# mpieva/mapping-iterative-assembler

Hardware: NVIDIA B200
Metric: aligned reads/sec per iteration (windowed PSSM DP + traceback + score cut + consensus) (higher is better)
Workload: dtype int32

## Files before the change

include/miagpu.h:

```cpp
#ifndef MIAGPU_H
#define MIAGPU_H

#include <stdint.h>

#ifdef __cplusplus
extern "C" {
#endif

#define MIAGPU_MAX_READ      256
#define MIAGPU_PSSM_INTS     775
#define MIAGPU_MAX_RUNS      24
#define MIAGPU_NBUCKET       10
#define MIAGPU_COUNTS_PER_COL 10

#define MIAGPU_RUN_M 0
#define MIAGPU_RUN_I 1
#define MIAGPU_RUN_D 2
#define MIAGPU_RUN_TYPE(x) ((x) >> 14)
#define MIAGPU_RUN_LEN(x)  ((x) & 0x3fff)

#define MIAGPU_ST_OK          0
#define MIAGPU_ST_RUNS_OVERFLOW 1
#define MIAGPU_ST_SKIPPED     2
#define MIAGPU_ST_STR_OVERFLOW 4
// ... 208 lines not shown
  const uint16_t* packed;
  const uint8_t* unique_best;
  const uint8_t* dropped_front;
  const uint8_t* dropped_back;
  const int64_t* fsdb_order;
} miagpu_maln_reads;

int miagpu_maln_ref_size( int ref_len, int circular );
int miagpu_write_maln( const char* path, const miagpu_maln_header* hd,
                       const miagpu_maln_reads* rd, int64_t* n_alnseqs_out );

int miagpu_write_maln_fsdb( miagpu_ctx* ctx, const char* path, const miagpu_maln_header* hd,
                            const miagpu_maln_reads* rd, int64_t* n_alnseqs_out );

#define MIAGPU_MISINC_INTS 1116
int miagpu_misincorporation( miagpu_ctx* ctx, int64_t* counts );

int miagpu_last_buckets( miagpu_ctx* ctx, int32_t* k, int32_t* reads,
                         int64_t* cells, float* ms );
#define MIAGPU_NPAIRCLASS 8
int miagpu_last_pair_buckets( miagpu_ctx* ctx, int32_t* k, int32_t* reads, int32_t* pairs,
                              int64_t* cells, float* ms, int32_t* fallback_reads,
                              int32_t* max_len16 );
int miagpu_last_timing( miagpu_ctx* ctx, float* ms_kernels, float* ms_h2d,
                        float* ms_d2h, int64_t* dp_cells, int32_t* launches );
int miagpu_int32_peak( miagpu_ctx* ctx, double* ops_per_s );
void* miagpu_stream( miagpu_ctx* ctx );

#ifdef __cplusplus
}
#endif
#endif
```

mapping-iterative-assembler_b200/api.py:

```python
import ctypes as C
import os

import numpy as np

HERE = os.path.dirname(os.path.abspath(__file__))
LIB_PATH = os.environ.get("MIAGPU_LIB") or os.path.join(HERE, "libmiagpu.so")
MAX_RUNS = 24
RUN_M, RUN_I, RUN_D = 0, 1, 2
MISINC_SHAPE = (31, 6, 6)
MISINC_CODES = "ACGTN-"

_i32p = C.POINTER(C.c_int32)
_u8p = C.POINTER(C.c_uint8)
_u16p = C.POINTER(C.c_uint16)
_i64p = C.POINTER(C.c_int64)


class MiaGpuError(RuntimeError):
    pass


ENTRY_DTYPE = np.dtype([("read", np.int32), ("col_begin", np.int32), ("col_count", np.int32), ("ref_pos", np.int32),
                        ("front_len", np.int32), ("total_len", np.int32), ("act_bias", np.int32), ("dropped", np.uint8),
                        ("back_formula", np.uint8), ("reserved", np.uint8, 2)])
# ... 40 lines not shown
    L.miagpu_score_cut.argtypes = [C.c_int64, C.c_void_p, C.c_void_p, C.c_void_p, C.POINTER(C.c_double), C.POINTER(C.c_double)]
    L.miagpu_cull_flags.argtypes = [C.c_int64, C.c_void_p, C.c_void_p, C.c_void_p, C.c_int, C.c_int, C.c_double, C.c_double, C.c_void_p]
    L.miagpu_set_alignment_inputs.argtypes = [C.c_void_p, C.c_void_p, C.c_void_p, C.c_void_p]
    L.miagpu_realign_resident.argtypes = [C.c_void_p]
    L.miagpu_adopt_alignment.argtypes = [C.c_void_p, C.c_void_p, C.c_void_p, C.c_void_p]
    L.miagpu_set_cut_inputs.argtypes = [C.c_void_p, C.c_void_p, C.c_void_p, C.c_void_p]
    L.miagpu_reset_dropped.argtypes = [C.c_void_p]
    L.miagpu_iterate_resident.argtypes = [C.c_void_p, C.c_int, C.c_int, C.c_double, C.c_double, C.c_int, C.POINTER(C.c_double),
                                          C.POINTER(C.c_double), C.c_void_p, C.c_void_p, C.c_void_p, _i32p]
    L.miagpu_last_buckets.argtypes = [C.c_void_p, C.c_void_p, C.c_void_p, C.c_void_p, C.c_void_p]
    L.miagpu_iterate_host.argtypes = ([C.c_void_p, C.c_int64] + [C.c_void_p] * 12 + [C.c_int64, _i64p, C.c_void_p, C.c_void_p, C.c_int, C.c_int,
                                      C.c_double, C.c_double, C.c_void_p, C.c_int, C.c_void_p, C.c_char_p, _i32p])
    _vpp = C.POINTER(C.c_void_p)
    L.miagpu_shard_begin.argtypes = [C.c_void_p, C.c_int, C.c_int, C.c_int64, C.c_int, C.c_int, C.c_double, C.c_double, _vpp, _i64p]
    L.miagpu_shard_begin_host.argtypes = ([C.c_void_p, C.c_int, C.c_int, C.c_int64, C.c_int64] + [C.c_void_p] * 14 +
                                          [C.c_int, C.c_int, C.c_double, C.c_double, _vpp, _i64p])
    L.miagpu_shard_fit.argtypes = [C.c_void_p, _vpp, _vpp, _i64p]
    L.miagpu_shard_cut.argtypes = [C.c_void_p, C.POINTER(C.c_double), C.POINTER(C.c_double), _vpp, _i64p]
    L.miagpu_shard_finish.argtypes = [C.c_void_p, C.c_int, C.c_void_p, C.c_void_p, C.c_int64, _i64p, C.c_void_p, C.c_char_p, _i32p]
    L.miagpu_last_cut_stats.argtypes = [C.c_void_p, _i64p, _i64p]
    L.miagpu_trim.argtypes = [C.c_void_p, C.c_int64, C.c_void_p, C.c_void_p, C.c_char_p, C.c_int] + [C.c_void_p] * 6
    L.miagpu_repeat_filter.argtypes = [C.c_void_p, C.c_int64] + [C.c_void_p] * 5 + [C.c_int, C.c_int, C.c_void_p, C.c_void_p]
    L.miagpu_last_pair_buckets.argtypes = [C.c_void_p] + [C.c_void_p] * 5 + [_i32p, _i32p]
    L.miagpu_last_timing.argtypes = [C.c_void_p, C.POINTER(C.c_float), C.POINTER(C.c_float), C.POINTER(C.c_float), _i64p, _i32p]
    L.miagpu_int32_peak.argtypes = [C.c_void_p, C.POINTER(C.c_double)]
    L.miagpu_get_alignment.argtypes = [C.c_void_p] + [C.c_void_p] * 6
    L.miagpu_align_windows.argtypes = [C.c_void_p] + [C.c_void_p] * 3 + [C.c_int] + [C.c_void_p] * 7
    L.miagpu_fastx_open.argtypes = [_vpp, C.c_char_p]
    L.miagpu_fastx_open_memory.argtypes = [_vpp, C.c_void_p, C.c_int64]
    L.miagpu_fastx_format.argtypes = [C.c_void_p]
    L.miagpu_fastx_next.argtypes = [C.c_void_p, C.c_int64, _i64p]
    L.miagpu_fastx_batch.argtypes = [C.c_void_p] + [_vpp] * 7
    L.miagpu_fastx_close.argtypes = [C.c_void_p]
    L.miagpu_fastx_close.restype = None
    L.miagpu_maln_ref_size.argtypes = [C.c_int, C.c_int]
    L.miagpu_read_pssm.argtypes = [C.c_char_p, _i32p]
    L.miagpu_write_maln.argtypes = [C.c_char_p, C.c_void_p, C.c_void_p, _i64p]
    L.miagpu_write_maln_fsdb.argtypes = [C.c_void_p, C.c_char_p, C.c_void_p, C.c_void_p, _i64p]
    L.miagpu_set_fsdb.argtypes = [C.c_void_p] + [C.c_void_p] * 6 + [C.c_int64, C.c_void_p, C.c_int]
    L.miagpu_get_fsdb.argtypes = [C.c_void_p] + [C.c_void_p] * 6 + [_i64p]
    L.miagpu_last_fsdb_stats.argtypes = [C.c_void_p, _i64p, _i64p, _i64p, _i64p]
    L.miagpu_distant_retry.argtypes = [C.c_void_p, _i64p, _i64p]
    L.miagpu_distant_retry_begin.argtypes = [C.c_void_p, _i64p, _i32p]
    L.miagpu_distant_retry_end.argtypes = [C.c_void_p, C.c_int, _i64p]
    L.miagpu_misincorporation.argtypes = [C.c_void_p, _i64p]
    L.miagpu_stream.restype = C.c_void_p
    L.miagpu_stream.argtypes = [C.c_void_p]
    _lib = L
    return L


EXPORTS = ["miagpu_device_count", "miagpu_create", "miagpu_destroy", "miagpu_last_error", "miagpu_version", "miagpu_set_pssm",
           "miagpu_get_pssm", "miagpu_set_reference", "miagpu_ref_wrap_len", "miagpu_build_kmers", "miagpu_upload_reads",
           "miagpu_pass1", "miagpu_last_pass1_stats", "miagpu_last_pass1_route", "miagpu_compact_reads", "miagpu_realign", "miagpu_realign_host", "miagpu_iterate_host", "miagpu_get_runs_packed",
           "miagpu_consensus", "miagpu_accumulate_gaps", "miagpu_accumulate_counts", "miagpu_call", "miagpu_consensus_natural", "miagpu_accumulate_gaps_natural",
           "miagpu_score_cut", "miagpu_cull_flags",
           "miagpu_set_alignment_inputs", "miagpu_realign_resident", "miagpu_adopt_alignment", "miagpu_set_cut_inputs", "miagpu_reset_dropped", "miagpu_iterate_resident", "miagpu_last_buckets", "miagpu_last_pair_buckets", "miagpu_last_timing",
           "miagpu_int32_peak", "miagpu_stream", "miagpu_shard_begin", "miagpu_shard_begin_host", "miagpu_shard_fit", "miagpu_shard_cut", "miagpu_shard_finish",
           "miagpu_last_cut_stats", "miagpu_repeat_filter", "miagpu_trim", "miagpu_get_alignment",
           "miagpu_fastx_open", "miagpu_fastx_open_memory", "miagpu_fastx_format", "miagpu_fastx_next", "miagpu_fastx_batch", "miagpu_fastx_close",
           "miagpu_maln_ref_size", "miagpu_write_maln", "miagpu_read_pssm", "miagpu_align_windows",
           "miagpu_set_fsdb", "miagpu_get_fsdb", "miagpu_last_fsdb_stats", "miagpu_distant_retry", "miagpu_write_maln_fsdb", "miagpu_last_pass1_cells", "miagpu_set_homopolymer", "miagpu_shard_flags", "miagpu_set_cons_capacity",
           "miagpu_distant_retry_begin", "miagpu_distant_retry_end", "miagpu_misincorporation"]


def _ptr(a):
    if a is None:
        return None
    if hasattr(a, "data_ptr"):
        return C.c_void_p(a.data_ptr())
    return C.c_void_p(a.ctypes.data)


class MiaGpu:

    def __init__(self, device=0):
        self.lib = load_library()
        h = C.c_void_p()
        if not self.lib.miagpu_create(C.byref(h), device):
            raise MiaGpuError(self.lib.miagpu_last_error().decode())
# ... 299 lines not shown
        return sc, a, e

    def get_alignment(self):
        out = {k: np.zeros(self.n, np.int32) for k in ("score", "as_out", "ae_out", "abr", "n_runs")}
        out["status"] = np.zeros(self.n, np.uint8)
        self._ck(self.lib.miagpu_get_alignment(self.h, *[_ptr(out[k]) for k in ("score", "as_out", "ae_out", "abr", "n_runs", "status")]))
        return out

    def realign_resident(self):
        self._ck(self.lib.miagpu_realign_resident(self.h))

    def last_buckets(self):
        k, r, cells, ms = np.zeros(10, np.int32), np.zeros(10, np.int32), np.zeros(10, np.int64), np.zeros(10, np.float32)
        self._ck(self.lib.miagpu_last_buckets(self.h, _ptr(k), _ptr(r), _ptr(cells), _ptr(ms)))
        return [dict(K=int(k[i]), reads=int(r[i]), cells=int(cells[i]), ms=float(ms[i])) for i in range(10) if r[i]]

    def last_pair_buckets(self):
        k, r, pr = np.zeros(8, np.int32), np.zeros(8, np.int32), np.zeros(8, np.int32)
        cells, ms = np.zeros(8, np.int64), np.zeros(8, np.float32)
        fb, ml = C.c_int32(), C.c_int32()
        self._ck(self.lib.miagpu_last_pair_buckets(self.h, _ptr(k), _ptr(r), _ptr(pr), _ptr(cells), _ptr(ms), C.byref(fb), C.byref(ml)))
        return ([dict(K=int(k[i]), reads=int(r[i]), pairs=int(pr[i]), cells=int(cells[i]), ms=float(ms[i])) for i in range(8) if r[i]],
                fb.value, ml.value)

    def accumulate_gaps(self, entries):
        entries = np.ascontiguousarray(entries, ENTRY_DTYPE)
        ptr, n = C.c_void_p(), C.c_int64()
        self._ck(self.lib.miagpu_accumulate_gaps(self.h, len(entries), _ptr(entries), C.byref(ptr), C.byref(n)))
        return ptr.value, n.value

    def accumulate_counts(self):
        ptr, n = C.c_void_p(), C.c_int64()
        self._ck(self.lib.miagpu_accumulate_counts(self.h, C.byref(ptr), C.byref(n)))
        return ptr.value, n.value

    def call(self, cons_code=1, want_counts=False, max_len=None):
        gaps = np.zeros(self.seq_len, np.int32)
        counts = np.zeros((self.seq_len, 10), np.int32) if want_counts else None
        buf = C.create_string_buffer(max_len or (self.seq_len * 4 + 4096))
        n = C.c_int32()
        self._ck(self.lib.miagpu_call(self.h, cons_code, _ptr(gaps), _ptr(counts), buf, C.byref(n)))
        return buf.value.decode(), gaps, counts

    def last_timing(self):
        k, h, d = C.c_float(), C.c_float(), C.c_float()
        cells, launches = C.c_int64(), C.c_int32()
# ... 147 lines not shown
```

mapping-iterative-assembler_b200/csrc/miagpu.cu:

```cuda
#include <stdarg.h>
#include <string.h>
#include <stdlib.h>

#include <algorithm>
#include <functional>
#include <chrono>
#include <thread>
#include <vector>

#include "common.cuh"
#include "realign.cuh"
#include "pair16.cuh"
#include "consensus.cuh"
#include "strip.cuh"
#include "pass1.cuh"
#include "sweep16.cuh"
#include "scorecut.hpp"
#include "scorecut.cuh"
#include "repeat.cuh"
#include "slots.cuh"
#include <unordered_map>
#include <cub/device/device_scan.cuh>
#include <cub/device/device_radix_sort.cuh>

namespace miagpu {

static thread_local char g_err[1024] = "";
void set_error(const char* fmt, ...) {
  va_list ap;
  va_start(ap, fmt);
  vsnprintf(g_err, sizeof(g_err), fmt, ap);
  va_end(ap);
}

template <typename T>
// ... 61 lines not shown
  DevBuf<uint16_t> d_runs;
  DevBuf<int32_t> d_meta;
  DevBuf<uint32_t> d_scratch[4];
  DevBuf<int32_t> d_p1trace;
  DevBuf<int32_t> d_sw_jobs, d_sw_layout, d_sw_pairs;
  DevBuf<int32_t> d_p1sunk;
  int p1_traced = 0, p1_swept = 0;
  bool hp = false, hps_valid = false;
  DevBuf<int32_t> d_hps[2];
  DevBuf<int32_t> d_ckh;
  cudaStream_t s_aux[4] = {};
  cudaEvent_t aev[8] = {};
  cudaStream_t launch_stream = nullptr;
  int launch_slot = 0;
  DevBuf<int16_t> d_prof16;
  DevBuf<uint8_t> d_kind;
  DevBuf<int32_t> d_pairs;
  int pssm_min = 0, pssm_max = 0, lmax16 = 0;
  cudaEvent_t pev[2 * P16_NKB] = {};
  float pair_ms[P16_NKB] = {};
  int32_t pair_reads[P16_NKB] = {}, pair_pairs[P16_NKB] = {};
  int64_t pair_cells[P16_NKB] = {};
  int32_t n_fallback = 0;
  int pair_g = 16;
  cudaStream_t s_up = nullptr, s_down = nullptr;
  cudaEvent_t cev[4 * 16] = {};
  cudaEvent_t xev[4] = {};
  int32_t* h_meta = nullptr;
  DevBuf<int32_t> d_seqlen;
  DevBuf<uint8_t> d_unique;
  DevBuf<CutStatsDev> d_cstats;
  DevBuf<CutTables> d_ctab;
  DevBuf<double> d_thr;
  DevBuf<CutBlockDev> d_cblk;
  struct CutHost* h_cut = nullptr;
  CutBlockDev* h_cblk = nullptr;
  int64_t h_cblk_cap = 0;
  char* h_call = nullptr;
  size_t h_call_cap = 0;
  int32_t* h_score = nullptr;
  int64_t h_score_cap = 0;
  std::vector<int32_t> h_seqlen;
  std::vector<uint8_t> h_unique;
  int64_t cut_inputs_n = -1;
  int64_t cut_serial_blocks = 0;
  DevBuf<int32_t> tr_prof, tr_ws, tr_wl, tr_out, tr_cnt;
// ... 329 lines not shown
  MIAGPU_CUDA(cudaSetDevice(c->device));
  if (n > 0x7fffffffLL / NBUCKET) { set_error("miagpu_upload_reads: at most %lld reads per batch", 0x7fffffffLL / NBUCKET); return 0; }
  int64_t total = n ? offsets[n] : 0;
  if (n && offsets[0] != 0) { set_error("miagpu_upload_reads: offsets[0] must be 0"); return 0; }
  if (!c->d_bases.reserve(total + 16) || !c->d_off.reserve(n + 1) || !reserve_per_read(c, n)) return 0;
  MIAGPU_CUDA(cudaEventRecord(c->ev[0], c->stream));
  if (n) {
    MIAGPU_CUDA(cudaMemcpyAsync(c->d_bases.p, bases, total, cudaMemcpyHostToDevice, c->stream));
    MIAGPU_CUDA(cudaMemcpyAsync(c->d_off.p, offsets, (n + 1) * sizeof(int64_t), cudaMemcpyHostToDevice, c->stream));
  }
  MIAGPU_CUDA(cudaEventRecord(c->ev[1], c->stream));
  MIAGPU_CUDA(cudaStreamSynchronize(c->stream));
  MIAGPU_CUDA(cudaEventElapsedTime(&c->ms_h2d, c->ev[0], c->ev[1]));
  c->n = n;
  c->total_bases = total;
  c->cut_inputs_n = -1;
  c->fs_on = false; c->fs_prev_valid = false;
  c->max_read_len = -1;
  return 1;
}

__global__ void classify_kernel(int64_t n, const int64_t* off, const int32_t* as, const int32_t* ae, int wrap_len, PairLmax lm,
                                int32_t* win_start, int32_t* win_len, int32_t* lists, uint8_t* kind, int32_t* meta, int explicit_win = 0,
                                const uint8_t* __restrict__ known = nullptr) {
  int lmax16 = 0;
  for (int k = 0; k < P16_NKB; k++) lmax16 = max(lmax16, lm.v[k]);
  __shared__ int s_cnt[NBUCKET], s_base[NBUCKET], s_maxL[NBUCKET], s_pop[NBUCKET];
  __shared__ unsigned long long s_cells[NBUCKET];
  __shared__ int s_hist[P16_KEYS];
  __shared__ int s_preads[P16_NKB], s_pmaxl[P16_NKB];
  __shared__ unsigned long long s_pcells[P16_NKB];
  if (threadIdx.x < NBUCKET) { s_cnt[threadIdx.x] = 0; s_maxL[threadIdx.x] = 0; s_pop[threadIdx.x] = 0; s_cells[threadIdx.x] = 0; }
  if (threadIdx.x < P16_NKB) { s_preads[threadIdx.x] = 0; s_pcells[threadIdx.x] = 0; s_pmaxl[threadIdx.x] = 0; }
  if (lmax16 > 0) for (int i = threadIdx.x; i < P16_KEYS; i += blockDim.x) s_hist[i] = 0;
  __syncthreads();
  int64_t i = (int64_t)blockIdx.x * blockDim.x + threadIdx.x;
  const int lane = threadIdx.x & 31;
  const unsigned lt = (1u << lane) - 1;
  int b = -1, slot = 0, L = 0, key = -1, kb = -1;
  unsigned cells = 0;
  bool direct = false;
  if (i < n && known && !known[i]) {
    kind[i] = 15;
  } else if (i < n) {
    L = (int)(off[i + 1] - off[i]);
    int rs = as[i] - REALIGN_BUFFER < 0 ? 0 : as[i] - REALIGN_BUFFER;
    int re = (ae[i] + REALIGN_BUFFER + 1 > wrap_len) ? wrap_len : ae[i] + REALIGN_BUFFER;
    bool whole = rs + L > re;
    if (whole) { rs = 0; re = wrap_len; }
    if (explicit_win) { rs = as[i]; re = ae[i]; whole = true; }
    int len1 = re - rs;
    win_start[i] = rs;
    win_len[i] = len1;
    b = bucket32_of(len1);
    if (L <= 0 || L > MAX_READ) b = NBUCKET - 1;
    kb = p16_class(len1);
    const bool elig = b != NBUCKET - 1 && kb >= 0 && !whole && L <= lm.v[kb < 0 ? 0 : kb];
    cells = (unsigned)max(L, 0) * (unsigned)len1;
    if (elig) { kind[i] = (uint8_t)(16 + kb); key = kb * (P16_MAXL + 1) + L; }
    else { kind[i] = (uint8_t)b; direct = true; kb = -1; }
  }
  {
    const unsigned peers = __match_any_sync(0xffffffffu, b);
    const int mx = __reduce_max_sync(peers, L);
    const unsigned long long cs = (unsigned long long)__reduce_add_sync(peers, cells & 0xffffu) +
                                  ((unsigned long long)__reduce_add_sync(peers, cells >> 16) << 16);
    if (b >= 0 && (peers & lt) == 0) {
      atomicAdd(&s_pop[b], __popc(peers));
      atomicMax(&s_maxL[b], mx);
      atomicAdd(&s_cells[b], cs);
    }
  }
  if (lmax16 > 0) {
    const unsigned pk = __match_any_sync(0xffffffffu, key);
    if (key >= 0 && (pk & lt) == 0) atomicAdd(&s_hist[key], __popc(pk));
    const unsigned pc = __match_any_sync(0xffffffffu, kb);
    const unsigned long long cs = (unsigned long long)__reduce_add_sync(pc, cells & 0xffffu) + ((unsigned long long)__reduce_add_sync(pc, cells >> 16) << 16);
    const int mxl = __reduce_max_sync(pc, L);
    if (kb >= 0 && (pc & lt) == 0) { atomicAdd(&s_preads[kb], __popc(pc)); atomicAdd(&s_pcells[kb], cs); atomicMax(&s_pmaxl[kb], mxl); }
  }
  {
    const int db = direct ? b : -1;
    const unsigned pd = __match_any_sync(0xffffffffu, db);
    int base = 0;
    if (direct && (pd & lt) == 0) base = atomicAdd(&s_cnt[b], __popc(pd));
    base = __shfl_sync(0xffffffffu, base, __ffs(pd) - 1);
    slot = base + __popc(pd & lt);
  }
  __syncthreads();
  if (threadIdx.x < NBUCKET) {
    const int t = threadIdx.x;
    s_base[t] = s_cnt[t] ? atomicAdd(&meta[META_COUNT + t], s_cnt[t]) : 0;
    if (s_maxL[t]) atomicMax(&meta[META_MAXL + t], s_maxL[t]);
    if (s_pop[t]) atomicAdd(&meta[META_POP + t], s_pop[t]);
    if (s_cells[t]) atomicAdd(reinterpret_cast<unsigned long long*>(meta + META_CELLS) + t, s_cells[t]);
  }
  if (threadIdx.x < P16_NKB && s_preads[threadIdx.x]) {
    atomicAdd(&meta[META_PREADS + threadIdx.x], s_preads[threadIdx.x]);
    atomicAdd(reinterpret_cast<unsigned long long*>(meta + META_PCELLS) + threadIdx.x, s_pcells[threadIdx.x]);
    atomicMax(&meta[META_PMAXL + threadIdx.x], s_pmaxl[threadIdx.x]);
  }
// ... 288 lines not shown
  int lmax16 = c->lmax16;
  if (const char* e = getenv("MIAGPU_PAIR16")) if (atoi(e) == 0) lmax16 = 0;
  c->pair_g = 16;
  PairLmax lm{};
  for (int kb = 0; kb < P16_NKB; kb++) lm.v[kb] = lmax16 > 0 ? std::min(p16_lmax(P16_COLS[kb] / realign_g(kb), c->pssm_max), P16_MAXL) : 0;
  return lm;
}
static bool pair_rb_class(miagpu_ctx* c, int kb, bool job) {
  if (const char* e = getenv("MIAGPU_PAIR_RB")) if (atoi(e) == 0) return false;
  if (realign_g(kb) != 16 || kb >= P16_NKB_WIDE || (job && kb < 2)) return false;
  return p16_rb_frame(P16_COLS[kb] / 16, c->pssm_max).room >= 16384;
}
static PairLmax pair_lmax(miagpu_ctx* c, bool job = false) {
  PairLmax lm = pair_lmax_low(c);
  for (int kb = 0; kb < P16_NKB; kb++)
    if (lm.v[kb] > 0 && pair_rb_class(c, kb, job)) lm.v[kb] = P16_MAXL;
  return lm;
}

static void realign_reset_stats(miagpu_ctx* c) {
  c->launches = 0;
  c->dp_cells = 0;
  c->n_fallback = 0;
  for (int kb = 0; kb < P16_NKB; kb++) { c->pair_ms[kb] = 0; c->pair_reads[kb] = 0; c->pair_pairs[kb] = 0; c->pair_cells[kb] = 0; }
  for (int b = 0; b < NBUCKET; b++) { c->bucket_ms[b] = 0; c->bucket_reads[b] = 0; c->bucket_cells[b] = 0; }
}

static int realign_classify(miagpu_ctx* c, const RealignJob& j, cudaStream_t st) {
  if (j.n == 0) return 1;
  PairLmax lm = pair_lmax(c);
  if (c->hp) for (int kb = 0; kb < P16_NKB; kb++) lm.v[kb] = 0;
  MIAGPU_CUDA(cudaMemsetAsync(j.d_meta, 0, META_WORDS * sizeof(int32_t), st));
  classify_kernel<<<(unsigned)((j.n + 255) / 256), 256, 0, st>>>(j.n, c->d_off.p + j.lo, c->d_as.p + j.lo, c->d_ae.p + j.lo, c->wrap_len, lm,
                                                                c->d_win_start.p + j.lo, c->d_win_len.p + j.lo, j.d_lists, c->d_kind.p + j.lo, j.d_meta,
                                                                c->explicit_windows ? 1 : 0, (c->fs_on && !c->explicit_windows) ? c->d_known.p + j.lo : nullptr);
  MIAGPU_CUDA(cudaGetLastError());
  c->launches++;
  if (lm.v[0] > 0) {
    pair_layout_kernel<<<1, LAYOUT_THREADS, 0, st>>>(j.d_meta, realign_np());
    MIAGPU_CUDA(cudaGetLastError());
    c->launches++;
  }
  MIAGPU_CUDA(cudaMemcpyAsync(j.h_meta, j.d_meta, sizeof(int32_t) * META_HOST, cudaMemcpyDeviceToHost, st));
  return 1;
}

static int realign_launch(miagpu_ctx* c, const RealignJob& j) {
  const int64_t n = j.n, lo = j.lo;
  if (n == 0) return 1;
  const int32_t* meta = j.h_meta;
  const PairNp npk = realign_np();
  const PairLmax lm_low = pair_lmax_low(c);
  const bool concurrent = !j.timed && !getenv("MIAGPU_SERIAL_LAUNCH") && !c->hp;
  int rr = 0;
  int64_t cells[NBUCKET], pcells[P16_NKB];
  memcpy(cells, meta + META_CELLS, sizeof(cells));
  memcpy(pcells, meta + META_PCELLS, sizeof(pcells));
  for (int b = 0; b < NBUCKET; b++) { c->bucket_cells[b] += cells[b]; c->dp_cells += cells[b]; }
// ... 121 lines not shown

static RealignJob whole_batch_job(miagpu_ctx* c) {
  RealignJob j;
  j.lo = 0; j.n = c->n; j.d_meta = c->d_meta.p; j.d_lists = c->d_lists.p; j.d_pairs = c->d_pairs.p; j.h_meta = c->h_meta; j.timed = true;
  return j;
}

static int realign_device(miagpu_ctx* c, bool timed = true) {
  realign_reset_stats(c);
  if (c->n == 0) return 1;
  RealignJob j = whole_batch_job(c);
  j.timed = timed;
  if (!realign_classify(c, j, c->stream)) return 0;
  MIAGPU_CUDA(cudaStreamSynchronize(c->stream));
  return realign_launch(c, j);
}

static int realign_bucket_times(miagpu_ctx* c) {
  if (c->n == 0) return 1;
  int32_t meta[META_HOST];
  MIAGPU_CUDA(cudaMemcpyAsync(meta, c->d_meta.p, sizeof(meta), cudaMemcpyDeviceToHost, c->stream));
  MIAGPU_CUDA(cudaStreamSynchronize(c->stream));
  c->n_fallback = meta[META_NFALL];
  int64_t cells32[NBUCKET];
  memcpy(cells32, meta + META_CELLS32, sizeof(cells32));
  for (int b = 0; b < NBUCKET; b++)
    if (c->bucket_reads[b]) {
      c->bucket_reads[b] = meta[META_COUNT + b];
      if (b != NBUCKET - 1) c->bucket_cells[b] = cells32[b];
      MIAGPU_CUDA(cudaEventElapsedTime(&c->bucket_ms[b], c->bev[2 * b], c->bev[2 * b + 1]));
    }
  for (int kb = 0; kb < P16_NKB; kb++)
    if (c->pair_pairs[kb]) MIAGPU_CUDA(cudaEventElapsedTime(&c->pair_ms[kb], c->pev[2 * kb], c->pev[2 * kb + 1]));
  return 1;
}

static int realign_common(miagpu_ctx* c, const uint8_t* rc, const int32_t* as, const int32_t* ae, int32_t* score,
                          int32_t* as_out, int32_t* ae_out, int32_t* abr, int32_t* n_runs, uint16_t* runs, uint8_t* status,
                          bool time_h2d_from_upload) {
  if (!c || !c->have_pssm || !c->have_ref) { set_error("miagpu_realign: set_pssm and set_reference first"); return 0; }
  misinc_invalidate(c, "a realign has replaced the alignments of that round");
  if (c->n && (!rc || !as || !ae)) { set_error("miagpu_realign: rc/as/ae are required"); return 0; }
  MIAGPU_CUDA(cudaSetDevice(c->device));
  const int64_t n = c->n;
  MIAGPU_CUDA(cudaEventRecord(c->ev[0], c->stream));
  if (n) {
// ... 70 lines not shown

extern "C" int miagpu_last_buckets(miagpu_ctx* c, int32_t* k, int32_t* reads, int64_t* cells, float* ms) {
  if (!c) { set_error("miagpu_last_buckets: NULL ctx"); return 0; }
  for (int b = 0; b < NBUCKET; b++) {
    if (k) k[b] = BUCKET_K[b];
    if (reads) reads[b] = c->bucket_reads[b];
    if (cells) cells[b] = c->bucket_cells[b];
    if (ms) ms[b] = c->bucket_ms[b];
  }
  return 1;
}

extern "C" int miagpu_last_pair_buckets(miagpu_ctx* c, int32_t* k, int32_t* reads, int32_t* pairs, int64_t* cells, float* ms, int32_t* fallback_reads, int32_t* max_len16) {
  if (!c) { set_error("miagpu_last_pair_buckets: NULL ctx"); return 0; }
  for (int kb = 0; kb < P16_NKB_WIDE; kb++) {
    if (k) k[kb] = P16_COLS[kb] / realign_g(kb);
    if (reads) reads[kb] = c->pair_reads[kb];
    if (pairs) pairs[kb] = c->pair_pairs[kb];
    if (cells) cells[kb] = c->pair_cells[kb];
    if (ms) ms[kb] = c->pair_ms[kb];
  }
  if (fallback_reads) *fallback_reads = c->n_fallback;
  if (max_len16) *max_len16 = c->lmax16;
  return 1;
}

extern "C" int miagpu_set_alignment_inputs(miagpu_ctx* c, const uint8_t* rc, const int32_t* as, const int32_t* ae) {
  if (!c || (c->n && (!rc || !as || !ae))) { set_error("miagpu_set_alignment_inputs: bad argument"); return 0; }
  misinc_invalidate(c, "miagpu_set_alignment_inputs has replaced the strands of that round's reads");
  MIAGPU_CUDA(cudaSetDevice(c->device));
  if (c->n) {
    MIAGPU_CUDA(cudaMemcpyAsync(c->d_rc.p, rc, c->n, cudaMemcpyHostToDevice, c->stream));
    MIAGPU_CUDA(cudaMemcpyAsync(c->d_as.p, as, c->n * 4, cudaMemcpyHostToDevice, c->stream));
    MIAGPU_CUDA(cudaMemcpyAsync(c->d_ae.p, ae, c->n * 4, cudaMemcpyHostToDevice, c->stream));
  }
  MIAGPU_CUDA(cudaStreamSynchronize(c->stream));
  c->h_rc.assign(rc, rc + c->n);
  return 1;
}

extern "C" int miagpu_adopt_alignment(miagpu_ctx* c, int32_t* score, int32_t* as, int32_t* ae) {
  if (!c) { set_error("miagpu_adopt_alignment: no context"); return 0; }
  MIAGPU_CUDA(cudaSetDevice(c->device));
  const int64_t n = c->n;
  if (n) {
    MIAGPU_CUDA(cudaMemcpyAsync(c->d_as.p, c->d_as_out.p, n * 4, cudaMemcpyDeviceToDevice, c->stream));
// ... 1279 lines not shown
    if (tr.on && k == 0) MIAGPU_CUDA(cudaEventRecord(c->ev[6], main));
    if (!realign_launch(c, j)) return 0;
    if (tr.on && k == C - 1) MIAGPU_CUDA(cudaEventRecord(c->ev[7], main));
    MIAGPU_CUDA(cudaEventRecord(c->cev[4 * k + 1], main));
    if (stats && !cut_launch_stats(c, j.lo, j.lo + j.n, unique_best != nullptr)) return 0;
    MIAGPU_CUDA(cudaStreamWaitEvent(down, c->cev[4 * k + 1], 0));
    MIAGPU_CUDA(cudaMemcpyAsync(score + j.lo, c->d_score.p + j.lo, j.n * 4, cudaMemcpyDeviceToHost, down));
    MIAGPU_CUDA(cudaEventRecord(c->cev[4 * k + 2], down));
    if (as_out) MIAGPU_CUDA(cudaMemcpyAsync(as_out + j.lo, c->d_as_out.p + j.lo, j.n * 4, cudaMemcpyDeviceToHost, down));
    if (ae_out) MIAGPU_CUDA(cudaMemcpyAsync(ae_out + j.lo, c->d_ae_out.p + j.lo, j.n * 4, cudaMemcpyDeviceToHost, down));
    if (abr) MIAGPU_CUDA(cudaMemcpyAsync(abr + j.lo, c->d_abr.p + j.lo, j.n * 4, cudaMemcpyDeviceToHost, down));
    if (n_runs) MIAGPU_CUDA(cudaMemcpyAsync(n_runs + j.lo, c->d_nruns.p + j.lo, j.n * 4, cudaMemcpyDeviceToHost, down));
    if (status) MIAGPU_CUDA(cudaMemcpyAsync(status + j.lo, c->d_status.p + j.lo, j.n, cudaMemcpyDeviceToHost, down));
  }
  tr.mark("DP + downloads enqueued");
  return 1;
}
static int host_round_stats(miagpu_ctx* c, int C) {
  c->ms_h2d = 0; c->ms_kernels = 0; c->ms_d2h = 0;
  for (int k = 0; k < C; k++) {
    int32_t nf = 0;
    MIAGPU_CUDA(cudaMemcpy(&nf, c->d_meta.p + (size_t)META_WORDS * k + META_NFALL, 4, cudaMemcpyDeviceToHost));
    c->n_fallback += nf;
  }
  return 1;
}

extern "C" int miagpu_iterate_host(miagpu_ctx* c, int64_t n, const uint8_t* bases, const int64_t* offsets, const uint8_t* rc,
                                   const int32_t* as, const int32_t* ae, int32_t* score, int32_t* as_out, int32_t* ae_out,
                                   int32_t* abr, int32_t* n_runs, uint8_t* status, uint16_t* packed_runs, int64_t capacity,
                                   int64_t* total_runs, const int32_t* seq_len, const uint8_t* unique_best, int hard_cut,
                                   int score_cut_set, double slope, double intercept, uint8_t* dropped, int cons_code,
                                   int32_t* gaps_out, char* cons_out, int32_t* cons_len) {
  const bool fit = !score_cut_set && hard_cut <= 0;
  const Trace tr;
  int C = 1;
  if (!host_round_front(c, "miagpu_iterate_host", n, bases, offsets, rc, as, ae, score, as_out, ae_out, abr, n_runs, status, seq_len,
                        unique_best, fit, dropped, tr, &C)) {
    if (c && c->s_up) { cudaStreamSynchronize(c->s_down); cudaStreamSynchronize(c->s_up); }
    return 0;
  }
  cudaStream_t down = c->s_down, up = c->s_up;
  IterTail t{};
  t.h_seq_len = seq_len; t.h_unique = unique_best; t.h_score = score; t.scores_on_host = c->cev[4 * (C - 1) + 2];
  t.wait_old_flags = true;
  t.hard_cut = hard_cut; t.score_cut_set = score_cut_set; t.slope = slope; t.intercept = intercept; t.cons_code = cons_code;
// ... 61 lines not shown
  }
  MIAGPU_CUDA(cudaEventRecord(c->ev[1], main));
  cut_init_kernel<<<1, 256, 0, main>>>(c->d_cstats.p);
  MIAGPU_CUDA(cudaGetLastError());
  if (!realign_device(c, false)) return 0;
  MIAGPU_CUDA(cudaEventRecord(c->ev[2], main));
  if (fit) {
    MIAGPU_CUDA(cudaStreamWaitEvent(down, c->ev[2], 0));
    MIAGPU_CUDA(cudaMemcpyAsync(c->h_score, c->d_score.p, n * 4, cudaMemcpyDeviceToHost, down));
    MIAGPU_CUDA(cudaEventRecord(c->cev[2], down));
    if (!cut_launch_stats(c, 0, n, !c->h_unique.empty())) return 0;
  }
  tr.mark("DP enqueued");
  IterTail t{};
  t.h_seq_len = c->h_seqlen.data(); t.h_unique = c->h_unique.empty() ? nullptr : c->h_unique.data(); t.h_score = c->h_score;
  t.scores_on_host = c->cev[2]; t.wait_old_flags = false;
  t.hard_cut = hard_cut; t.score_cut_set = score_cut_set; t.slope = slope; t.intercept = intercept; t.cons_code = cons_code;
  t.dropped = dropped; t.gaps_out = gaps_out; t.cons_out = cons_out; t.cons_len = cons_len;
  t.slope_out = slope_out; t.intercept_out = intercept_out;
  if (!iterate_tail(c, t, tr)) { cudaStreamSynchronize(down); return 0; }
  MIAGPU_CUDA(cudaEventElapsedTime(&c->ms_kernels, c->ev[1], c->ev[2]));
  c->ms_h2d = c->ms_d2h = 0;
  MIAGPU_CUDA(cudaMemcpy(&c->n_fallback, c->d_meta.p + META_NFALL, 4, cudaMemcpyDeviceToHost));
  if (c->fs_on) {
    c->fs_prev_seq_len = c->seq_len;
    fs_carry_submat(c);
  }
  c->misinc_stale = nullptr;
  return 1;
}

static int shard_reserve(miagpu_ctx* c, int world, int64_t n_max) {
  const int64_t nb = (n_max + CUT_BLOCK - 1) / CUT_BLOCK;
  const int64_t words = (nb * (int64_t)sizeof(ShardBlockRec) + 3) / 4 + (SHARD_PF_SLOTS + 8) + (int64_t)SHARD_PF_SLOTS * CUT_BLOCK;
  c->sh_stride = (words + 3) / 4 * 4;
  c->sh_nb = nb;
  if (!c->d_sh_send.reserve(c->sh_stride) || !c->d_sh_recv.reserve((size_t)world * c->sh_stride) || !c->d_sh_prep.reserve(1) || !cut_reserve(c, nb * CUT_BLOCK)) return 0;
  const size_t need = (size_t)world * c->sh_stride * sizeof(uint32_t);
  if (c->h_sh_cap < need) {
    if (c->h_sh_recv) cudaFreeHost(c->h_sh_recv);
    c->h_sh_recv = nullptr; c->h_sh_cap = 0;
    MIAGPU_CUDA(cudaMallocHost(&c->h_sh_recv, need + need / 8));
    c->h_sh_cap = need + need / 8;
  }
  return 1;
}
// ... 271 lines not shown
  c->cons_stage = 2;
  const int launches = c->launches;
  if (!miagpu_call(c, cons_code, gaps_out, nullptr, cons_out, cons_len)) { cudaStreamSynchronize(down); return 0; }
  c->launches = launches + 1;
  float ms_dp = 0;
  if (!c->sh_host) MIAGPU_CUDA(cudaEventElapsedTime(&ms_dp, c->ev[1], c->ev[2]));
  if (packed_runs || total_runs) {
    int64_t tot = 0;
    const int l2 = c->launches;
    if (!miagpu_get_runs_packed(c, nullptr, packed_runs, capacity, &tot)) { cudaStreamSynchronize(down); return 0; }
    c->launches = l2 + 4;
    if (total_runs) *total_runs = tot;
  }
  MIAGPU_CUDA(cudaStreamSynchronize(down));
  if (c->sh_host) {
    MIAGPU_CUDA(cudaStreamSynchronize(c->s_up));
    if (!host_round_stats(c, c->sh_chunks)) return 0;
    c->misinc_stale = nullptr;
    return 1;
  }
  c->ms_kernels = ms_dp;
  c->ms_h2d = c->ms_d2h = 0;
  MIAGPU_CUDA(cudaMemcpy(&c->n_fallback, c->d_meta.p + META_NFALL, 4, cudaMemcpyDeviceToHost));
  if (c->fs_on) c->fs_prev_seq_len = c->seq_len;
  c->misinc_stale = nullptr;
  return 1;
}

extern "C" int miagpu_shard_flags(miagpu_ctx* c, void** flag_buf, int64_t* bytes) {
  if (!c) { set_error("miagpu_shard_flags: no context"); return 0; }
  if (flag_buf) *flag_buf = c->fs_on ? c->d_slot_flag.p : nullptr;
  if (bytes) *bytes = c->fs_on ? c->fs_slot_cap : 0;
  return 1;
}

extern "C" int miagpu_last_cut_stats(miagpu_ctx* c, int64_t* serial_blocks, int64_t* fetched_blocks) {
  if (!c) { set_error("miagpu_last_cut_stats: no context"); return 0; }
  if (serial_blocks) *serial_blocks = c->cut_serial_blocks;
  if (fetched_blocks) *fetched_blocks = c->sh_fetched;
  return 1;
}

__global__ void trim_codes_kernel(int64_t total, uint8_t* bases_to_codes) {
  const int64_t i = (int64_t)blockIdx.x * blockDim.x + threadIdx.x;
  if (i < total) bases_to_codes[i] = (uint8_t)base_code(bases_to_codes[i]);
}
// ... 744 lines not shown
```

mapping-iterative-assembler_b200/csrc/pair16.cuh:

```cuda
#pragma once
#include "common.cuh"
#include "realign.cuh"
#include <type_traits>

namespace miagpu {

constexpr int P16_MAXL = MAX_READ;
constexpr int PROF16_N = 2 * NMAT * 5 * PROF_ROW_INTS;
constexpr int P16_NKB = 12;
constexpr int P16_NKB_WIDE = 8;
constexpr int P16_TAB_WORDS = 64;

__host__ __device__ constexpr int p16_off(int K) { return 32768 - 2 * GOP - GEP - PSSM_ABS_LIMIT - GEP * K - 32; }
__host__ __device__ inline int p16_lmax(int K, int max_entry) {
  const int inc = max_entry + GEP;
  return inc > 0 ? (32767 + p16_off(K) - GEP * (K - 2)) / inc : MAX_READ;
}
__host__ __device__ inline int p16_class(int len1) {
  return len1 <= 128 ? 0 : len1 <= 144 ? 1 : len1 <= 160 ? 2 : len1 <= 176 ? 3 : len1 <= 192 ? 4 : len1 <= 208 ? 5 : len1 <= 224 ? 6 : len1 <= 256 ? 7 : -1;
}
__host__ __device__ inline int p16_job_class(int len1) {
  return len1 <= 64 ? 8 : len1 <= 80 ? 9 : len1 <= 96 ? 10 : len1 <= 112 ? 11 : p16_class(len1);
}
__host__ __device__ inline int bucket32_of(int len1) {
  return len1 <= 64 ? 0 : len1 <= 128 ? 1 : len1 <= 160 ? 2 : len1 <= 192 ? 3 : len1 <= 224 ? 4 : len1 <= 256 ? 5 : len1 <= 320 ? 6 : len1 <= 384 ? 7 : len1 <= 512 ? 8 : 9;
}

struct PairLmax { int v[P16_NKB]; };

constexpr int META_COUNT = 0;
constexpr int META_WORK = 16;
constexpr int META_MAXL = 32;
constexpr int META_CELLS = 48;
constexpr int META_POP = 80;
constexpr int META_NPAIRS = 96;
constexpr int META_PWORK = 108;
constexpr int META_PREADS = 120;
constexpr int META_PCELLS = 132;
constexpr int META_MAXLEN = 156;
constexpr int META_NFALL = 157;
constexpr int META_P1 = 158;
constexpr int META_CELLS32 = 168;
constexpr int META_PMAXL = 192;
constexpr int META_HOST = 208;
constexpr int P16_KEYS = P16_NKB * (P16_MAXL + 1);
constexpr int META_KEYS = 3200;
constexpr int META_HIST = 256;
constexpr int META_PSTART = META_HIST + META_KEYS;
constexpr int META_CURSOR = META_PSTART + META_KEYS;
constexpr int META_WORDS = META_CURSOR + META_KEYS;
static_assert(P16_KEYS <= META_KEYS && P16_NKB == 12 && META_PCELLS % 2 == 0, "meta layout");

struct Pair16Params {
  const uint8_t* bases;
  const int64_t* off;
  const uint8_t* rc;
  const int32_t* win_start;
  const int32_t* win_len;
  int32_t* win_len_narrow;
  const int32_t* pairs;
  const int32_t* n_items;
  int32_t* counter;
  const uint8_t* ref_codes;
  int32_t ref_bytes;
  int32_t ref_in_smem;
// ... 418 lines not shown
```

Measured before the change: 255.8 million.

## Add ungapped-diagonal prefilter that settles reads before full DP

Adds a warp-per-read kernel that runs before classification. It scores ungapped diagonals against the PSSM and prunes candidate diagonals with a suffix upper bound over the first rows. When only a few diagonals survive and the best one beats a bound on any gapped alignment, it writes the ungapped alignment directly and marks the read so the classifier skips the banded DP for it. This is meant to avoid full DP and traceback for reads whose best alignment provably has no gaps, at the cost of an extra launch and scan per iteration for reads that still go to DP.

New measurement: 425.6 million, median of 6. +66.4%, better.

```diff
diff --git a/include/miagpu.h b/include/miagpu.h
--- a/include/miagpu.h
+++ b/include/miagpu.h
@@ -254,6 +254,7 @@
 int miagpu_last_pair_buckets( miagpu_ctx* ctx, int32_t* k, int32_t* reads, int32_t* pairs,
                               int64_t* cells, float* ms, int32_t* fallback_reads,
                               int32_t* max_len16 );
+int miagpu_last_diag_settled( miagpu_ctx* ctx, int32_t* settled_reads );
 int miagpu_last_timing( miagpu_ctx* ctx, float* ms_kernels, float* ms_h2d,
                         float* ms_d2h, int64_t* dp_cells, int32_t* launches );
 int miagpu_int32_peak( miagpu_ctx* ctx, double* ops_per_s );
diff --git a/mapping-iterative-assembler_b200/api.py b/mapping-iterative-assembler_b200/api.py
--- a/mapping-iterative-assembler_b200/api.py
+++ b/mapping-iterative-assembler_b200/api.py
@@ -86,6 +86,7 @@
     L.miagpu_trim.argtypes = [C.c_void_p, C.c_int64, C.c_void_p, C.c_void_p, C.c_char_p, C.c_int] + [C.c_void_p] * 6
     L.miagpu_repeat_filter.argtypes = [C.c_void_p, C.c_int64] + [C.c_void_p] * 5 + [C.c_int, C.c_int, C.c_void_p, C.c_void_p]
     L.miagpu_last_pair_buckets.argtypes = [C.c_void_p] + [C.c_void_p] * 5 + [_i32p, _i32p]
+    L.miagpu_last_diag_settled.argtypes = [C.c_void_p, _i32p]
     L.miagpu_last_timing.argtypes = [C.c_void_p, C.POINTER(C.c_float), C.POINTER(C.c_float), C.POINTER(C.c_float), _i64p, _i32p]
     L.miagpu_int32_peak.argtypes = [C.c_void_p, C.POINTER(C.c_double)]
     L.miagpu_get_alignment.argtypes = [C.c_void_p] + [C.c_void_p] * 6
@@ -119,7 +120,7 @@
            "miagpu_pass1", "miagpu_last_pass1_stats", "miagpu_last_pass1_route", "miagpu_compact_reads", "miagpu_realign", "miagpu_realign_host", "miagpu_iterate_host", "miagpu_get_runs_packed",
            "miagpu_consensus", "miagpu_accumulate_gaps", "miagpu_accumulate_counts", "miagpu_call", "miagpu_consensus_natural", "miagpu_accumulate_gaps_natural",
            "miagpu_score_cut", "miagpu_cull_flags",
-           "miagpu_set_alignment_inputs", "miagpu_realign_resident", "miagpu_adopt_alignment", "miagpu_set_cut_inputs", "miagpu_reset_dropped", "miagpu_iterate_resident", "miagpu_last_buckets", "miagpu_last_pair_buckets", "miagpu_last_timing",
+           "miagpu_set_alignment_inputs", "miagpu_realign_resident", "miagpu_adopt_alignment", "miagpu_set_cut_inputs", "miagpu_reset_dropped", "miagpu_iterate_resident", "miagpu_last_buckets", "miagpu_last_pair_buckets", "miagpu_last_diag_settled", "miagpu_last_timing",
            "miagpu_int32_peak", "miagpu_stream", "miagpu_shard_begin", "miagpu_shard_begin_host", "miagpu_shard_fit", "miagpu_shard_cut", "miagpu_shard_finish",
            "miagpu_last_cut_stats", "miagpu_repeat_filter", "miagpu_trim", "miagpu_get_alignment",
            "miagpu_fastx_open", "miagpu_fastx_open_memory", "miagpu_fastx_format", "miagpu_fastx_next", "miagpu_fastx_batch", "miagpu_fastx_close",
@@ -465,6 +466,11 @@
         self._ck(self.lib.miagpu_last_pair_buckets(self.h, _ptr(k), _ptr(r), _ptr(pr), _ptr(cells), _ptr(ms), C.byref(fb), C.byref(ml)))
         return ([dict(K=int(k[i]), reads=int(r[i]), pairs=int(pr[i]), cells=int(cells[i]), ms=float(ms[i])) for i in range(8) if r[i]],
                 fb.value, ml.value)
+
+    def last_diag_settled(self):
+        v = C.c_int32()
+        self._ck(self.lib.miagpu_last_diag_settled(self.h, C.byref(v)))
+        return v.value
 
     def accumulate_gaps(self, entries):
         entries = np.ascontiguousarray(entries, ENTRY_DTYPE)
diff --git a/mapping-iterative-assembler_b200/csrc/diag.cuh b/mapping-iterative-assembler_b200/csrc/diag.cuh
--- /dev/null
+++ b/mapping-iterative-assembler_b200/csrc/diag.cuh
@@ -0,0 +1,160 @@
+#pragma once
+#include "common.cuh"
+#include "realign.cuh"
+
+namespace miagpu {
+
+constexpr uint8_t DIAG_KIND = 14;
+constexpr int DIAG_MAXW = 256;
+constexpr int DIAG_PER_LANE = DIAG_MAXW / 32;
+constexpr int DIAG_SWEEP_ROWS = 32;
+constexpr int DIAG_SURVIVORS = 2;
+
+struct DiagParams {
+  int64_t n;
+  const int64_t* off;
+  const uint8_t* bases;
+  const uint8_t* rc;
+  const int32_t* as;
+  const int32_t* ae;
+  const uint8_t* known;
+  int32_t wrap_len;
+  const uint8_t* ref_codes;
+  const int32_t* prof;
+  int32_t* score;
+  int32_t* as_out;
+  int32_t* ae_out;
+  int32_t* abr;
+  int32_t* n_runs;
+  uint16_t* runs;
+  uint8_t* status;
+  uint8_t* kind;
+  int32_t* n_settled;
+};
+
+__global__ void __launch_bounds__(WARPS_PER_BLOCK * 32) diag_kernel(DiagParams p) {
+  __shared__ int s_prof[PROF_INTS];
+  __shared__ int s_mx[2 * NMAT * 5];
+  __shared__ uint8_t s_win[WARPS_PER_BLOCK][DIAG_MAXW];
+  __shared__ uint16_t s_ro[WARPS_PER_BLOCK][MAX_READ];
+  __shared__ int s_R[WARPS_PER_BLOCK][MAX_READ + 1];
+  for (int t = threadIdx.x; t < PROF_INTS; t += blockDim.x) s_prof[t] = p.prof[t];
+  __syncthreads();
+  for (int t = threadIdx.x; t < 2 * NMAT * 5; t += blockDim.x) {
+    const int* e = s_prof + t * PROF_ROW_INTS;
+    s_mx[t] = max(max(max(e[0], e[1]), max(e[2], e[3])), e[4]);
+  }
+  __syncthreads();
+  const int lane = threadIdx.x & 31, warp = threadIdx.x >> 5;
+  uint8_t* win = s_win[warp];
+  uint16_t* ro = s_ro[warp];
+  int* R = s_R[warp];
+  int settled = 0;
+  const int64_t stride = (int64_t)gridDim.x * WARPS_PER_BLOCK;
+  for (int64_t i = (int64_t)blockIdx.x * WARPS_PER_BLOCK + warp; i < p.n; i += stride) {
+    const int64_t o = p.off[i];
+    const int L = (int)(p.off[i + 1] - o);
+    const int rs = max(p.as[i] - REALIGN_BUFFER, 0);
+    const int re = p.ae[i] + REALIGN_BUFFER + 1 > p.wrap_len ? p.wrap_len : p.ae[i] + REALIGN_BUFFER;
+    const int W = re - rs;
+    bool ok = L >= 1 && L <= MAX_READ && rs + L <= re && W <= DIAG_MAXW && (!p.known || p.known[i]);
+    if (ok) {
+      const int s = p.rc[i] ? 1 : 0;
+      const int CH = (L + 31) >> 5;
+      const int r0 = lane * CH;
+      int msum = 0, neg = 0, mmin = INT_MAX;
+      for (int q = 0; q < CH; q++) {
+        const int r = r0 + q;
+        if (r < L) {
+          const int ri = prof_row_index(s, sm_depth(r, L), base_code(p.bases[o + r]));
+          ro[r] = (uint16_t)ri;
+          const int m = s_mx[ri / PROF_ROW_INTS];
+          msum += m; neg += min(0, m + GEP); mmin = min(mmin, m + GEP);
+        }
+      }
+      for (int c = lane; c < W; c += 32) win[c] = p.ref_codes[rs + c];
+      int suf = msum;
+#pragma unroll
+      for (int d = 1; d < 32; d <<= 1) {
+        const int y = __shfl_down_sync(0xffffffffu, suf, d);
+        if (lane + d < 32) suf += y;
+      }
+      __syncwarp();
+      {
+        int run = suf;
+        for (int q = 0; q < CH; q++) {
+          const int r = r0 + q;
+          if (r < L) { R[r] = run; run -= s_mx[ro[r] / PROF_ROW_INTS]; }
+        }
+        if (lane == 0) R[L] = 0;
+      }
+      const int U = __shfl_sync(0xffffffffu, suf, 0);
+      neg = (int)__reduce_add_sync(0xffffffffu, (unsigned)neg);
+      mmin = __reduce_min_sync(0xffffffffu, mmin);
+      const int Bgap = U - GOP - min(GEP, neg < 0 ? neg : mmin);
+      __syncwarp();
+      auto diag_sum = [&](int d) {
+        int v = 0;
+        for (int q = 0; q < CH; q++) {
+          const int r = r0 + q;
+          if (r < L) v += s_prof[ro[r] + win[d + r]];
+        }
+        return (int)__reduce_add_sync(0xffffffffu, (unsigned)v);
+      };
+      const int nd = W - L + 1;
+      const int dh = min(max(p.as[i] - rs, 0), nd - 1);
+      int best = diag_sum(dh), bd = dh;
+      const int T = max(Bgap, best - 1);
+      const int kn = (nd + 31) >> 5;
+      int pre[DIAG_PER_LANE];
+      unsigned alive = 0;
+#pragma unroll
+      for (int k = 0; k < DIAG_PER_LANE; k++) {
+        pre[k] = 0;
+        const int d = lane + 32 * k;
+        if (d < nd && d != dh) alive |= 1u << k;
+      }
+      int live = (int)__reduce_add_sync(0xffffffffu, __popc(alive));
+      const int rows = min(L, DIAG_SWEEP_ROWS);
+      for (int r = 0; r < rows && live > DIAG_SURVIVORS; r++) {
+        const int ri = ro[r], Rn = R[r + 1];
+#pragma unroll
+        for (int k = 0; k < DIAG_PER_LANE; k++) {
+          if (k < kn && ((alive >> k) & 1u)) {
+            pre[k] += s_prof[ri + win[lane + 32 * k + r]];
+            if (pre[k] + Rn <= T) alive &= ~(1u << k);
+          }
+        }
+        live = (int)__reduce_add_sync(0xffffffffu, __popc(alive));
+      }
+      ok = live <= DIAG_SURVIVORS;
+      while (ok) {
+        const unsigned lanes = __ballot_sync(0xffffffffu, alive != 0);
+        if (!lanes) break;
+        const int src = __ffs(lanes) - 1;
+        const int k = __shfl_sync(0xffffffffu, __ffs(alive) - 1, src);
+        if (lane == src) alive &= alive - 1;
+        const int d = src + 32 * k;
+        const int v = diag_sum(d);
+        if (v > best || (v == best && d < bd)) { best = v; bd = d; }
+      }
+      ok = ok && best > Bgap;
+      if (ok && lane == 0) {
+        const int aec = bd + L - 1;
+        p.score[i] = best;
+        p.as_out[i] = bd + rs;
+        p.ae_out[i] = aec + rs;
+        p.abr[i] = 0;
+        p.n_runs[i] = 1;
+        p.runs[i * MAX_RUNS] = (uint16_t)((MIAGPU_RUN_M << 14) | L);
+        p.status[i] = MIAGPU_ST_OK;
+        settled++;
+      }
+      __syncwarp();
+    }
+    if (lane == 0) p.kind[i] = ok ? DIAG_KIND : 0;
+  }
+  if (lane == 0 && settled) atomicAdd(p.n_settled, settled);
+}
+
+}
diff --git a/mapping-iterative-assembler_b200/csrc/miagpu.cu b/mapping-iterative-assembler_b200/csrc/miagpu.cu
--- a/mapping-iterative-assembler_b200/csrc/miagpu.cu
+++ b/mapping-iterative-assembler_b200/csrc/miagpu.cu
@@ -11,6 +11,7 @@
 #include "common.cuh"
 #include "realign.cuh"
 #include "pair16.cuh"
+#include "diag.cuh"
 #include "consensus.cuh"
 #include "strip.cuh"
 #include "pass1.cuh"
@@ -118,6 +119,7 @@
   int32_t pair_reads[P16_NKB] = {}, pair_pairs[P16_NKB] = {};
   int64_t pair_cells[P16_NKB] = {};
   int32_t n_fallback = 0;
+  int32_t n_diag = 0;
   int pair_g = 16;
   cudaStream_t s_up = nullptr, s_down = nullptr;
   cudaEvent_t cev[4 * 16] = {};
@@ -493,7 +495,7 @@
 
 __global__ void classify_kernel(int64_t n, const int64_t* off, const int32_t* as, const int32_t* ae, int wrap_len, PairLmax lm,
                                 int32_t* win_start, int32_t* win_len, int32_t* lists, uint8_t* kind, int32_t* meta, int explicit_win = 0,
-                                const uint8_t* __restrict__ known = nullptr) {
+                                const uint8_t* __restrict__ known = nullptr, int diag = 0) {
   int lmax16 = 0;
   for (int k = 0; k < P16_NKB; k++) lmax16 = max(lmax16, lm.v[k]);
   __shared__ int s_cnt[NBUCKET], s_base[NBUCKET], s_maxL[NBUCKET], s_pop[NBUCKET];
@@ -508,7 +510,7 @@
   int64_t i = (int64_t)blockIdx.x * blockDim.x + threadIdx.x;
   const int lane = threadIdx.x & 31;
   const unsigned lt = (1u << lane) - 1;
-  int b = -1, slot = 0, L = 0, key = -1, kb = -1;
+  int b = -1, slot = 0, L = 0, key = -1, kb = -1, pL = 0;
   unsigned cells = 0;
   bool direct = false;
   if (i < n && known && !known[i]) {
@@ -528,7 +530,8 @@
     kb = p16_class(len1);
     const bool elig = b != NBUCKET - 1 && kb >= 0 && !whole && L <= lm.v[kb < 0 ? 0 : kb];
     cells = (unsigned)max(L, 0) * (unsigned)len1;
-    if (elig) { kind[i] = (uint8_t)(16 + kb); key = kb * (P16_MAXL + 1) + L; }
+    if (diag && kind[i] == DIAG_KIND) { if (!elig) kb = -1; }
+    else if (elig) { kind[i] = (uint8_t)(16 + kb); key = kb * (P16_MAXL + 1) + L; pL = L; }
     else { kind[i] = (uint8_t)b; direct = true; kb = -1; }
   }
   {
@@ -547,7 +550,7 @@
     if (key >= 0 && (pk & lt) == 0) atomicAdd(&s_hist[key], __popc(pk));
     const unsigned pc = __match_any_sync(0xffffffffu, kb);
     const unsigned long long cs = (unsigned long long)__reduce_add_sync(pc, cells & 0xffffu) + ((unsigned long long)__reduce_add_sync(pc, cells >> 16) << 16);
-    const int mxl = __reduce_max_sync(pc, L);
+    const int mxl = __reduce_max_sync(pc, pL);
     if (kb >= 0 && (pc & lt) == 0) { atomicAdd(&s_preads[kb], __popc(pc)); atomicAdd(&s_pcells[kb], cs); atomicMax(&s_pmaxl[kb], mxl); }
   }
   {
@@ -882,8 +885,32 @@
   c->launches = 0;
   c->dp_cells = 0;
   c->n_fallback = 0;
+  c->n_diag = 0;
   for (int kb = 0; kb < P16_NKB; kb++) { c->pair_ms[kb] = 0; c->pair_reads[kb] = 0; c->pair_pairs[kb] = 0; c->pair_cells[kb] = 0; }
   for (int b = 0; b < NBUCKET; b++) { c->bucket_ms[b] = 0; c->bucket_reads[b] = 0; c->bucket_cells[b] = 0; }
+}
+
+static bool diag_stage_on(miagpu_ctx* c) {
+  if (c->hp || c->explicit_windows) return false;
+  const char* e = getenv("MIAGPU_DIAG");
+  return !(e && atoi(e) == 0);
+}
+static int launch_diag(miagpu_ctx* c, const RealignJob& j, const uint8_t* known, cudaStream_t st) {
+  static int per_sm_d[MAX_DEVICES];
+  int& per_sm = per_sm_d[c->device % MAX_DEVICES];
+  if (!per_sm) MIAGPU_CUDA(cudaOccupancyMaxActiveBlocksPerMultiprocessor(&per_sm, diag_kernel, WARPS_PER_BLOCK * 32, 0));
+  if (per_sm < 1) { set_error("diag_kernel does not fit on an SM"); return 0; }
+  DiagParams p{};
+  p.n = j.n; p.off = c->d_off.p + j.lo; p.bases = c->d_bases.p; p.rc = c->d_rc.p + j.lo; p.as = c->d_as.p + j.lo; p.ae = c->d_ae.p + j.lo;
+  p.known = known; p.wrap_len = c->wrap_len; p.ref_codes = c->d_ref.p; p.prof = c->d_prof.p;
+  p.score = c->d_score.p + j.lo; p.as_out = c->d_as_out.p + j.lo; p.ae_out = c->d_ae_out.p + j.lo; p.abr = c->d_abr.p + j.lo;
+  p.n_runs = c->d_nruns.p + j.lo; p.runs = c->d_runs.p + j.lo * MAX_RUNS; p.status = c->d_status.p + j.lo;
+  p.kind = c->d_kind.p + j.lo; p.n_settled = j.d_meta + META_NDIAG;
+  const int blocks = (int)std::min<int64_t>((int64_t)c->num_sms * per_sm, (j.n + WARPS_PER_BLOCK - 1) / WARPS_PER_BLOCK);
+  diag_kernel<<<blocks, WARPS_PER_BLOCK * 32, 0, st>>>(p);
+  MIAGPU_CUDA(cudaGetLastError());
+  c->launches++;
+  return 1;
 }
 
 static int realign_classify(miagpu_ctx* c, const RealignJob& j, cudaStream_t st) {
@@ -891,9 +918,12 @@
   PairLmax lm = pair_lmax(c);
   if (c->hp) for (int kb = 0; kb < P16_NKB; kb++) lm.v[kb] = 0;
   MIAGPU_CUDA(cudaMemsetAsync(j.d_meta, 0, META_WORDS * sizeof(int32_t), st));
+  const uint8_t* known = (c->fs_on && !c->explicit_windows) ? c->d_known.p + j.lo : nullptr;
+  const bool diag = diag_stage_on(c);
+  if (diag && !launch_diag(c, j, known, st)) return 0;
   classify_kernel<<<(unsigned)((j.n + 255) / 256), 256, 0, st>>>(j.n, c->d_off.p + j.lo, c->d_as.p + j.lo, c->d_ae.p + j.lo, c->wrap_len, lm,
                                                                 c->d_win_start.p + j.lo, c->d_win_len.p + j.lo, j.d_lists, c->d_kind.p + j.lo, j.d_meta,
-                                                                c->explicit_windows ? 1 : 0, (c->fs_on && !c->explicit_windows) ? c->d_known.p + j.lo : nullptr);
+                                                                c->explicit_windows ? 1 : 0, known, diag ? 1 : 0);
   MIAGPU_CUDA(cudaGetLastError());
   c->launches++;
   if (lm.v[0] > 0) {
@@ -1061,6 +1091,7 @@
   MIAGPU_CUDA(cudaMemcpyAsync(meta, c->d_meta.p, sizeof(meta), cudaMemcpyDeviceToHost, c->stream));
   MIAGPU_CUDA(cudaStreamSynchronize(c->stream));
   c->n_fallback = meta[META_NFALL];
+  c->n_diag = meta[META_NDIAG];
   int64_t cells32[NBUCKET];
   memcpy(cells32, meta + META_CELLS32, sizeof(cells32));
   for (int b = 0; b < NBUCKET; b++)
@@ -1177,6 +1208,12 @@
   }
   if (fallback_reads) *fallback_reads = c->n_fallback;
   if (max_len16) *max_len16 = c->lmax16;
+  return 1;
+}
+
+extern "C" int miagpu_last_diag_settled(miagpu_ctx* c, int32_t* settled_reads) {
+  if (!c || !settled_reads) { set_error("miagpu_last_diag_settled: NULL argument"); return 0; }
+  *settled_reads = c->n_diag;
   return 1;
 }
 
@@ -2502,6 +2539,8 @@
     int32_t nf = 0;
     MIAGPU_CUDA(cudaMemcpy(&nf, c->d_meta.p + (size_t)META_WORDS * k + META_NFALL, 4, cudaMemcpyDeviceToHost));
     c->n_fallback += nf;
+    MIAGPU_CUDA(cudaMemcpy(&nf, c->d_meta.p + (size_t)META_WORDS * k + META_NDIAG, 4, cudaMemcpyDeviceToHost));
+    c->n_diag += nf;
   }
   return 1;
 }
@@ -2609,6 +2648,7 @@
   MIAGPU_CUDA(cudaEventElapsedTime(&c->ms_kernels, c->ev[1], c->ev[2]));
   c->ms_h2d = c->ms_d2h = 0;
   MIAGPU_CUDA(cudaMemcpy(&c->n_fallback, c->d_meta.p + META_NFALL, 4, cudaMemcpyDeviceToHost));
+  MIAGPU_CUDA(cudaMemcpy(&c->n_diag, c->d_meta.p + META_NDIAG, 4, cudaMemcpyDeviceToHost));
   if (c->fs_on) {
     c->fs_prev_seq_len = c->seq_len;
     fs_carry_submat(c);
@@ -2926,6 +2966,7 @@
   c->ms_kernels = ms_dp;
   c->ms_h2d = c->ms_d2h = 0;
   MIAGPU_CUDA(cudaMemcpy(&c->n_fallback, c->d_meta.p + META_NFALL, 4, cudaMemcpyDeviceToHost));
+  MIAGPU_CUDA(cudaMemcpy(&c->n_diag, c->d_meta.p + META_NDIAG, 4, cudaMemcpyDeviceToHost));
   if (c->fs_on) c->fs_prev_seq_len = c->seq_len;
   c->misinc_stale = nullptr;
   return 1;
diff --git a/mapping-iterative-assembler_b200/csrc/pair16.cuh b/mapping-iterative-assembler_b200/csrc/pair16.cuh
--- a/mapping-iterative-assembler_b200/csrc/pair16.cuh
+++ b/mapping-iterative-assembler_b200/csrc/pair16.cuh
@@ -41,6 +41,7 @@
 constexpr int META_NFALL = 157;
 constexpr int META_P1 = 158;
 constexpr int META_CELLS32 = 168;
+constexpr int META_NDIAG = 188;
 constexpr int META_PMAXL = 192;
 constexpr int META_HOST = 208;
 constexpr int P16_KEYS = P16_NKB * (P16_MAXL + 1);
```
